# robotvisionmu/DenseMonoSLAM

Hardware: AMD Instinct MI355X
Metric: frames/sec ICP+RGB+fusion @640x480 (higher is better)
Workload: dtype f32; 1 GPU; TUM fr1/desk-like 640x480 full 3-level ICP+RGB tracking (SO3 + {10,5,4} GN iterations) + surfel index-map fusion; synthetic box-room RGB-D stream, loop closure off (--o), NID keyframing off (--nkf); cameras_per_gpu=1, n_pred=2, n_pred_project_passes=1, surfels_per_map=246557, surfels_total=246557, exchange=none (1 camera)

## Files before the change

densemonoslam_amd/capi.py:

```python
import ctypes as C
import os

import numpy as np

_HERE = os.path.dirname(os.path.abspath(__file__))
LIB_PATH = os.environ.get("DMS_LIB_PATH") or os.path.join(_HERE, "libdmslam_hip.so")

if not os.path.exists(LIB_PATH):
    raise ImportError(
        "densemonoslam_amd: %s is missing — build it with `make` (hipcc --offload-arch=gfx950) "
        "or `python -c 'import __graft_entry__ as g; g.build()'`; there is no CPU fallback" % LIB_PATH
    )

lib = C.CDLL(LIB_PATH)

DMS_OK = 0
NUM_PYRS = 3
MAX_SENSORS = 8


class Image2D(C.Structure):
    _fields_ = [("data", C.c_void_p), ("pitch", C.c_size_t), ("rows", C.c_int), ("cols", C.c_int)]


# ... 203 lines not shown
lib.dms_pyrDownGaussF.argtypes = [_I2, _I2, _P]
lib.dms_pyrDownUcharGauss.argtypes = [_I2, _I2, _P]
lib.dms_computeDerivativeImages.argtypes = [_I2, _I2, _I2, _P]
lib.dms_nid_workspace_bytes.argtypes = [C.c_int]
lib.dms_nid_workspace_bytes.restype = C.c_size_t
lib.dms_computeNIDImg.argtypes = [_I2, _I2, _I2, _I2, _I2, C.c_int, _P, C.c_size_t, C.POINTER(C.c_float), _P]
lib.dms_computeNIDDepth.argtypes = [_I2, _I2, _I2, C.c_int, C.c_float, _P, C.c_size_t, C.POINTER(C.c_float), _P]

lib.dms_fusion_wait_frame_done.argtypes = [_P, _P]
lib.dms_fusion_set_tracker_budget.argtypes = [_P, _I, _I]
lib.dms_fusion_get_tracker_budget.argtypes = [_P, C.POINTER(C.c_int), C.POINTER(C.c_int)]
lib.dms_fusion_allow_late_frame.argtypes = [_P, _I]
lib.dms_odometry_set_resident_budget.argtypes = [_P, _I, _I]
lib.dms_odometry_get_resident_budget.argtypes = [_P, C.POINTER(C.c_int), C.POINTER(C.c_int)]
lib.dms_exact_arith_selftest.argtypes = [_I, _F, C.POINTER(C.c_ulonglong), C.POINTER(C.c_uint)]

lib.dms_odometry_create.argtypes = [C.POINTER(_P), _I, _I, _F, _F, _F, _F, _F, _F]
lib.dms_odometry_destroy.argtypes = [_P]
lib.dms_odometry_set_mode.argtypes = [_P, _I, _I, _I, _I]
lib.dms_odometry_set_exec.argtypes = [_P, _I, _I, _I]
lib.dms_odometry_inject_timeout.argtypes = [_P, _I]
lib.dms_odometry_debug_set.argtypes = [_P, C.c_char_p, _I]
lib.dms_odometry_canon_retries.argtypes = [_P, _IP]
lib.dms_odometry_get_mode.argtypes = [_P, _IP, _IP, _IP]
lib.dms_odometry_get_level_shape.argtypes = [_P, _I, _IP, _IP, _IP]
lib.dms_debug_scalar_gn.argtypes = [_P, _P, _F, _P, _P, _P, _F, _F, _F, _F, _I, _P, _P, _P, _P, _P, _P]
lib.dms_debug_scalar_so3.argtypes = [_P, _P, _P, _F, _F, _F, _F, _P, _P, _P]
lib.dms_odometry_initICP_depth.argtypes = [_P, _I2, _F, _P]
lib.dms_odometry_initICP_maps.argtypes = [_P, _P, _P, _F, _P]
lib.dms_odometry_initICPModel.argtypes = [_P, _P, _P, _F, _FP, _P]
lib.dms_odometry_initRGB.argtypes = [_P, _I2, _P]
lib.dms_odometry_initRGBModel.argtypes = [_P, _I2, _P]
lib.dms_odometry_initFirstRGB.argtypes = [_P, _I2, _P]
lib.dms_odometry_initModelFused.argtypes = [_P, _P, _P, _P, _P, _P, _P, _P, C.c_int, _P, _P]
lib.dms_odometry_getIncrementalTransformation.argtypes = [_P, _FP, _FP, _I, _F, _I, _I, _I, _I, C.POINTER(TrackResult), _P]
lib.dms_odometry_track_async.argtypes = [_P, _FP, _FP, _I, _F, _I, _I, _I, _I, _P]
lib.dms_odometry_fetch_result.argtypes = [_P, C.POINTER(TrackResult), _P]
lib.dms_odometry_getCovariance.argtypes = [_P, C.POINTER(C.c_double)]
lib.dms_odometry_get_buffer.argtypes = [_P, _I, _I, _I2]
lib.dms_odometry_set_profiling.argtypes = [_P, _I]
lib.dms_odometry_get_kernel_time.argtypes = [_P, C.c_char_p, C.POINTER(C.c_double), _IP]
```

densemonoslam_amd/csrc/canon.hpp:

```cpp
#pragma once
#include "common.hpp"

namespace dms {
namespace canon {

constexpr int kMargin = 6;
constexpr int kEmin = -40;
constexpr int kEmax = 100;
constexpr int kRetryStep = 8;
constexpr int kMaxRetries = 16;

__host__ __device__ __forceinline__ int exp_of(float d) {
  if (!(d > 0.f) || !(d < 3.0e38f)) return -127;
  int e;
  (void)frexpf(d, &e);
  return e;
}
__host__ __device__ __forceinline__ int clamp_e(int e) { return e < kEmin ? kEmin : (e > kEmax ? kEmax : e); }

template <int N>
struct Layout {
  static constexpr int NP = N * (N + 3) / 2;
  static constexpr int NV = NP + 2;
  static constexpr int SLOTS = NV > 16 ? 32 : 16;
// ... 141 lines not shown
template <int SL>
__device__ __forceinline__ double tree_rest(const double (&o1)[SL / 2]) {
  const int lane = threadIdx.x & 63;
  double o2[SL / 4];
#pragma unroll
  for (int m = 0; m < SL / 4; ++m) o2[m] = swap16_add(o1[2 * m], o1[2 * m + 1]);
  double o3[SL / 8];
#pragma unroll
  for (int m = 0; m < SL / 8; ++m) o3[m] = sel_add<8>(o2[2 * m], o2[2 * m + 1], (lane & 8) != 0);
  double r;
  if constexpr (SL == 32) {
    double o4[2];
#pragma unroll
    for (int m = 0; m < 2; ++m) o4[m] = sel_add<4>(o3[2 * m], o3[2 * m + 1], (lane & 4) != 0);
    r = sel_add<2>(o4[0], o4[1], (lane & 2) != 0);
  } else {
    r = sel_add<4>(o3[0], o3[1], (lane & 4) != 0);
    r += mov_xor<2>(r);
  }
  r += mov_xor<1>(r);
  return r;
}

template <int N, int P>
__device__ __forceinline__ double wave_sum(const float (&rows)[P][N + 1], const bool (&found)[P], const double (*s_bias)[32]) {
  using Lay = Layout<N>;
  constexpr int SL = Lay::SLOTS;
  const int lane = threadIdx.x & 63;
  const double* bias = s_bias[lane >> 5];
  double r64[P][N + 1];
#pragma unroll
  for (int p = 0; p < P; ++p)
#pragma unroll
    for (int c = 0; c <= N; ++c) r64[p][c] = (double)rows[p][c];
  constexpr int G = 4, NG = (Lay::NV + G - 1) / G;
  double o1[SL / 2];
#pragma unroll
  for (int m = 0; m < SL / 2; ++m) o1[m] = 0.0;
  double cur[G], nxt[G];
#pragma unroll
  for (int h = 0; h < G; ++h) cur[h] = h < Lay::NV ? bias[h] : 0.0;
  round_down_begin();
#pragma unroll
  for (int g = 0; g < NG; ++g) {
#pragma unroll
    for (int h = 0; h < G; ++h) nxt[h] = ((g + 1) * G + h < Lay::NV) ? bias[(g + 1) * G + h] : 0.0;
#pragma unroll
    for (int p = 0; p < P; ++p) {
#pragma unroll
      for (int h = 0; h < G; ++h) {
        const int k = g * G + h;
        if (k <= Lay::NP)
          cur[h] = fma_down(r64[p][Lay::vi(k)], r64[p][Lay::vj(k)], cur[h]);
        else if (k == Lay::NP + 1)
          cur[h] += found[p] ? 1.0 : 0.0;
      }
    }
#pragma unroll
    for (int h = 0; h < G; h += 2)
      if (g * G + h < Lay::NV) o1[(g * G + h) / 2] = swap32_add(cur[h], cur[h + 1]);
#pragma unroll
    for (int h = 0; h < G; ++h) cur[h] = nxt[h];
  }
  round_down_end();
  return tree_rest<SL>(o1);
}

template <int N>
__device__ __forceinline__ void acc_init(double (&acc)[Layout<N>::NV], const double (*s_bias)[32]) {
  const double* bias = s_bias[(threadIdx.x & 63) >> 5];
#pragma unroll
// ... 58 lines not shown
```

densemonoslam_amd/csrc/scan.hpp:

```cpp
#pragma once
#include <hip/hip_runtime.h>

namespace dms {

__device__ __forceinline__ unsigned block_sum_u32(unsigned v) {
  __shared__ unsigned s_w[4];
  __shared__ unsigned s_tot;
  const int lane = threadIdx.x & 63, wid = threadIdx.x >> 6;
  for (int off = 32; off > 0; off >>= 1) v += __shfl_down(v, off, 64);
  if (lane == 0) s_w[wid] = v;
  __syncthreads();
  if (threadIdx.x == 0) s_tot = s_w[0] + s_w[1] + s_w[2] + s_w[3];
  __syncthreads();
  const unsigned t = s_tot;
  __syncthreads();
  return t;
}

__device__ __forceinline__ unsigned block_exclusive_rank(bool flag, unsigned& total) {
  __shared__ unsigned s_w[4];
  const int lane = threadIdx.x & 63, wid = threadIdx.x >> 6;
  const unsigned long long mask = __ballot(flag);
  const unsigned below = __popcll(mask & ((1ull << lane) - 1ull));
  __syncthreads();
  if (lane == 0) s_w[wid] = __popcll(mask);
  __syncthreads();
  unsigned base = 0;
  for (int w = 0; w < wid; ++w) base += s_w[w];
  total = s_w[0] + s_w[1] + s_w[2] + s_w[3];
  return base + below;
}

static __global__ __launch_bounds__(1024) void k_scan_blocks(const unsigned* __restrict__ counts, unsigned* __restrict__ offsets, int nb,
                                                      unsigned* __restrict__ out_count, unsigned cap, unsigned* __restrict__ out_count2) {
  __shared__ unsigned s_w[16];
  __shared__ unsigned s_carry;
  const int lane = threadIdx.x & 63, wid = threadIdx.x >> 6;
  if (threadIdx.x == 0) s_carry = 0;
  __syncthreads();
  for (int base = 0; base < nb; base += 1024) {
    const int i = base + threadIdx.x;
    const unsigned v = i < nb ? counts[i] : 0u;
    unsigned incl = v;
    for (int off = 1; off < 64; off <<= 1) {
      const unsigned t = __shfl_up(incl, off, 64);
      if (lane >= off) incl += t;
    }
    if (lane == 63) s_w[wid] = incl;
    __syncthreads();
    unsigned wbase = 0;
    for (int w = 0; w < wid; ++w) wbase += s_w[w];
    const unsigned carry = s_carry;
// ... 61 lines not shown
```

densemonoslam_amd/csrc/track.hip:

```cpp
#include <hip/hip_ext.h>
#include <math.h>

#include <map>
#include <string>
#include <vector>

#include "internal.hpp"
#include "host_util.hpp"
#include "pixel_ops.hpp"
#include "smallmath.hpp"
#include "gn_scalar.hpp"
#include "canon.hpp"
#include "pyr_body.hpp"
#include "frame_state.hpp"
#include "track_init.hpp"
#include "model_bodies.hpp"
#include "surfel.hpp"
#include "resident_rule.hpp"
#include <mutex>

namespace dms {

constexpr bool kTrackerFma = true;

struct Buf {
  void* p = nullptr;
  size_t pitch = 0;
  int rows = 0, cols = 0;
  dms_image2d img() const {
    dms_image2d i;
    i.data = p;
    i.pitch = pitch;
    i.rows = rows;
    i.cols = cols;
    return i;
  }
};

}

using namespace dms;
// ... 27 lines not shown
  float cx, cy, fx, fy, distThres, angleThres;
  float sobelScale, maxDepthDeltaRGB, maxDepthRGB;
  float minGrad[DMS_NUM_PYRS];
  char* arena = nullptr;
  size_t arena_bytes = 0;
  Buf depth_tmp[3], vmaps_g_prev[3], nmaps_g_prev[3], vmaps_curr[3], nmaps_curr[3];
  Buf lastDepth[3], nextDepth[3], lastImage[3], nextImage[3], lastNextImage[3];
  Buf nextdIdx[3], nextdIdy[3], nextGate[3], pointClouds[3], corresImg[3];
  struct LiveSet {
    Buf depth_tmp[3], vmaps_curr[3], nmaps_curr[3], nextImage[3], nextdIdx[3], nextdIdy[3], nextGate[3];
  };
  LiveSet ring[3];
  char* ring_arena = nullptr;
  bool ring_enabled = false;
  const void* deriv_of = nullptr;
  float* vmaps_tmp = nullptr;
  float* nmaps_tmp = nullptr;
  long long* part_icp = nullptr;
  long long* part_rgb = nullptr;
  long long* part_so3 = nullptr;
  int* part_cnt = nullptr;
  unsigned* tickets = nullptr;
  unsigned long long* ar = nullptr;
  int first_delay = -1;
  bool long_levels_resident = true;
  int first_delay_lvl[4] = {-1, -1, -1, -1};
  int first_delay_for(int nb, int stage) const { return dms::first_delay_for(nb, stage >= 0 && stage < 4 ? first_delay_lvl[stage] : -1, first_delay); }
  int depth_bias = 0;
  int exp_bias = 0;
  long long* prof = nullptr;
  TrackState* state = nullptr;
  TrackState* host_state = nullptr;
  bool profiling = false;
  bool profiling_level0_only = false;
  StageClock clock;
};

namespace dms {

__global__ void k_track_init(TrackState* st, Prior prior, const float* __restrict__ prior_pose16, float fx, float fy, float cx, float cy,
                             int so3, int first_level, unsigned long long* sync_words, int n_sync, int inject_timeout, unsigned* zero16) {
  track_init_body(blockIdx.x, gridDim.x, threadIdx.x, blockDim.x, st, prior, prior_pose16, fx, fy, cx, cy, so3, first_level, sync_words, n_sync,
                  inject_timeout, zero16);
}

__global__ __launch_bounds__(256) void k_track_init_pyr(TrackState* st, Prior prior, const float* __restrict__ prior_pose16, float fx, float fy,
// ... 588 lines not shown
  }
  if (ICP) canon::next_exponents<6>(s_icp, st->E_icp);
  if (RGB) canon::next_exponents<6>(s_rgb, st->E_rgb);
  st->have_E = 1;
  st->canon_retries += retries;
}

constexpr int kPWaves = kPB / kWave;
constexpr unsigned kSpinLimit = 1u << 22;

struct LevelArgs {
  int n_iter, level, level_below;
  int rgbOnly;
  float icpWeight;
  float fx, fy, cx, cy;
  unsigned long long* ar;
  int first_delay;
  long long* prof;
  int early_exit;
  int finalize, fin_rgb;
  float* pose16_out;
  FrameState* frame;
  float weightMultiplier;
};

constexpr int kArShards = 8;
constexpr int kArStride = 64;
constexpr int kArPairBase = kArShards * kArStride;
constexpr int kArPairStride = 16;
constexpr int kArWords = kArPairBase + kArShards * kArPairStride;
constexpr int kArSlotCnt = 0, kArSlotSig = 1;
constexpr int kArPool = 6;
constexpr int kArSetsPerKernel = kArRing + kArPool;
constexpr int kArSets = 4 * kArSetsPerKernel;

__device__ __forceinline__ unsigned long long pair_pack(unsigned long long v) { return (1ull << 58) + v; }

__device__ __forceinline__ void poll_pause(int n) {
  for (int i = 0; i < n; ++i) __builtin_amdgcn_s_sleep(1);
}
template <int STRIDE>
__device__ __forceinline__ bool ar_wait(const unsigned long long* w, int slot, bool mine, int nb, unsigned long long& fld_out, int* timeout) {
  unsigned spins = 0;
  for (;;) {
    unsigned long long arr = 0, fld = 0;
    if (mine) {
// ... 13 lines not shown
    }
    ++spins;
    if (spins > kSpinLimit || ((spins & 1023u) == 0u && __hip_atomic_load(timeout, __ATOMIC_RELAXED, __HIP_MEMORY_SCOPE_AGENT) == 1)) {
      __hip_atomic_store(timeout, 1, __ATOMIC_RELAXED, __HIP_MEMORY_SCOPE_AGENT);
      fld_out = 0;
      return false;
    }
    __builtin_amdgcn_s_sleep(1);
  }
}
__device__ __forceinline__ long long ar_total(unsigned long long fld, int nb) { return (long long)fld - (long long)nb * (1ll << 52); }

__device__ __forceinline__ constexpr unsigned se3_diag_mask() {
  unsigned m = 0;
  for (int c = 0; c <= 6; ++c) m |= 1u << canon::Layout<6>::diag(c);
  return m;
}
__device__ __forceinline__ constexpr unsigned so3_diag_mask() {
  unsigned m = 0;
  for (int c = 0; c <= 3; ++c) m |= 1u << canon::Layout<3>::diag(c);
  return m;
}

template <bool ICP, bool RGB, int P, bool EXIT>
__device__ __forceinline__ void gn_level_body(TrackState* st, const GnArgs& a, const LevelArgs& L, const int nb) {
  constexpr bool kFma = kTrackerFma;
  __shared__ sc::GnLocal s;
  __shared__ int s_redi[kPWaves][2];
  __shared__ double s_red[kPWaves][32];
  __shared__ double s_red2[2][kPWaves][32];
  __shared__ double s_bias[2][2][32];
  __shared__ int s_E[2][8];
  __shared__ float s_sums[64];
  __shared__ double s_comb[28];
  __shared__ float s_held[48];
  __shared__ int s_none;
  __shared__ int s_done;
  __shared__ int s_cs[2];
  __shared__ int s_viol;
  __shared__ int s_retries;
  __shared__ sc::KPre s_k[2];
  const int tid = threadIdx.x;
  int eb_icp = 0, eb_rgb = 0;
  __shared__ long long s_prof[16];
  if (tid < 16) s_prof[tid] = 0;
  long long pc = L.prof ? wall_clock64() : 0;
  auto phase = [&](int i) {
    if (L.prof && blockIdx.x == 0 && tid == 0) {
      const long long now = wall_clock64();
      s_prof[i] += now - pc;
      pc = now;
    }
  };

  if (L.finalize && L.frame && blockIdx.x == 0 && tid >= 64 && tid < 80) s_held[16 + tid - 64] = L.frame->lastPose[tid - 64];
  if (L.finalize && L.frame && blockIdx.x == 0 && tid >= 80 && tid < 84) s_held[12 + tid - 80] = L.frame->cur.pose[12 + tid - 80];
  if (tid == 0) {
    s_none = 0;
    s_retries = 0;
    s_done = st->level_done[L.level];
    for (int i = 0; i < 16; ++i) s.resultRt[i] = st->resultRt[i];
    for (int i = 0; i < 9; ++i) {
      s.Rprev[i] = st->Rprev[i];
      s.Rprev_inv[i] = st->Rprev_inv[i];
      s.Rcurr[i] = st->Rcurr[i];
      s.krkinv[i] = st->krkinv[i];
    }
    for (int i = 0; i < 3; ++i) {
      s.tprev[i] = st->tprev[i];
      s.tcurr[i] = st->tcurr[i];
      s.kt[i] = st->kt[i];
    }
    s.lastRGBError = st->lastRGBError;
    s.lastRGBCount = st->lastRGBCount;
    s.lastICPError = st->lastICPError;
    s.lastICPCount = st->lastICPCount;
    s.iters_run = st->iters_run[L.level];
    for (int i = 0; i < 36; ++i) s.lastA[i] = st->lastA[i];
    for (int i = 0; i < 6; ++i) s.lastb[i] = st->lastb[i];
    level_exponents(st, a, true, s_E[0], s_E[1]);
    s_k[0] = sc::kpre_of(L.fx, L.fy, L.cx, L.cy, L.level);
    s_k[1] = sc::kpre_of(L.fx, L.fy, L.cx, L.cy, L.level_below);
  }

  const int N = a.cols * a.rows;
  int idx[P], px[P], py[P];
  IcpOwn io[P];
  RgbOwn ro[P];
  short gx[P], gy[P];
#pragma unroll
  for (int p = 0; p < P; ++p) {
    idx[p] = (blockIdx.x * P + p) * kPB + tid;
    const int ic = idx[p] < N ? idx[p] : idx[p] % N;
    py[p] = ic / a.cols;
    px[p] = ic - py[p] * a.cols;
    if (ICP) io[p] = icp_load_own(a.maps, px[p], py[p], a.rows);
    if (RGB) {
      ro[p] = rgb_load_own_gated(a.rgb, px[p], py[p]);
      gx[p] = trow(a.rgb.dIdx, a.rgb.dI_pitch, py[p])[px[p]];
      gy[p] = trow(a.rgb.dIdy, a.rgb.dI_pitch, py[p])[px[p]];
    }
  }
  const float invFx = 1.0f / a.fx, invFy = 1.0f / a.fy;
  __syncthreads();
  if (s_done) return;
  if (tid < 64) {
    canon::write_bias<6>(s_E[tid >> 5], s_bias[tid >> 5], tid & 31);
    eb_icp = canon::value_exp<6>(s_E[0], tid & 31);
    eb_rgb = canon::value_exp<6>(s_E[1], tid & 31);
  }
  __syncthreads();

  bool ended = false;
  int pool_used = 0;
  bool on_pool = false;
  phase(0);
  for (int it = 0; it < L.n_iter;) {
    IcpParams ip;
    RgbResParams rp;
    if (ICP) ip = icp_params_of(s.Rcurr, s.tcurr, s.Rprev_inv, s.tprev, a);
    if (RGB) rp = rgb_params_of(s.krkinv, s.kt, a);
    const float lastErr = (it == 0) ? 3.402823466e+38F : s.lastRGBError;

    IcpProj ir[P];
    RgbProj rr[P];
    IcpModel im[P];
    RgbModel rm[P];
#pragma unroll
    for (int p = 0; p < P; ++p) {
      if (ICP) {
        ir[p] = icp_project<kFma>(ip, io[p]);
        im[p] = icp_load_model(a.maps, ir[p], a.rows);
      }
      if (RGB) {
        rr[p] = rgb_project<kFma>(rp, ro[p], px[p], py[p]);
        rm[p] = rgb_load_model(a.rgb, rr[p]);
      }
    }
    float rows[P][7];
    bool found[P];
    int cnt = 0, sig = 0;
    dms_dataterm c[P];
#pragma unroll
    for (int p = 0; p < P; ++p) {
      const bool live = idx[p] < N;
      if (RGB) {
        int d2;
        const bool ok = rgb_finish(rp, ro[p], rr[p], rm[p], px[p], py[p], c[p], d2) && live;
        if (!live) c[p].valid = 0;
        if (ok) {
          cnt += 1;
          sig += d2;
        }
      }
      if (ICP) {
        found[p] = icp_finish<kFma>(ip, io[p], ir[p], im[p], rows[p]);
        if (!live) {
          found[p] = false;
#pragma unroll
          for (int k = 0; k < 7; ++k) rows[p][k] = 0.f;
        }
      }
    }
    phase(1);
    const bool stamp = L.prof && L.level == 0 && it == L.n_iter / 2 && tid == 0;
    if (stamp) L.prof[48 + blockIdx.x * 8 + 0] = wall_clock64();
    const size_t set = (size_t)(on_pool ? kArRing + pool_used - 1 : it % kArRing) * kArWords;
    unsigned long long* arw = L.ar + set + (size_t)(blockIdx.x & (kArShards - 1)) * kArStride;
    const unsigned long long* arp = L.ar + set;
    unsigned long long* arq = L.ar + set + kArPairBase + (size_t)(blockIdx.x & (kArShards - 1)) * kArPairStride;
    int rgbSize = 0, sigma = 0;
    if (RGB) {
      const int lane = tid & 63, wid = tid >> 6;
      cnt = wave_sum_to_lane63_i(cnt);
      sig = wave_sum_to_lane63_i(sig);
      if (lane == 63) {
        s_redi[wid][0] = cnt;
        s_redi[wid][1] = sig;
      }
      __syncthreads();
      if (tid < 64) {
        const int t = row8_sum_i(tid < 16 ? s_redi[tid & 7][tid >> 3] : 0);
        const unsigned long long cb = (unsigned long long)(unsigned)__builtin_amdgcn_readlane(t, 0);
        const unsigned long long sb = (unsigned long long)(unsigned)__builtin_amdgcn_readlane(t, 8);
        if (tid < 2) __hip_atomic_fetch_add(arq + tid, pair_pack(tid == kArSlotCnt ? cb : sb), __ATOMIC_RELAXED, __HIP_MEMORY_SCOPE_AGENT);
      }
    }
    phase(2);
    double r_icp = 0.0;
    if (ICP) {
      if (RGB) {
        r_icp = canon::wave_sum<6, P>(rows, found, s_bias[0]);
      } else {
        const double p_icp = canon::block_sum<6, P, kPWaves>(rows, found, s_bias[0], s_red);
        if (tid < kSE3) __hip_atomic_fetch_add(arw + tid, canon::pack_word(canon::to_units(p_icp, eb_icp)), __ATOMIC_RELAXED, __HIP_MEMORY_SCOPE_AGENT);
      }
    }
    f3 cpt[P];
    float cinvz[P];
    if (RGB) {
#pragma unroll
      for (int p = 0; p < P; ++p) {
        const float z = rm[p].d0;
        cpt[p] = mk3((((float)c[p].zero_x - a.cx) * z) * invFx, (((float)c[p].zero_y - a.cy) * z) * invFy, z);
        cinvz[p] = rgb_row_invz(cpt[p]);
      }
    }
    if (RGB) {
      if (tid < 64) {
        unsigned long long fld;
        if (stamp) L.prof[48 + blockIdx.x * 8 + 4] = wall_clock64();
        ar_wait<kArPairStride>(arp + kArPairBase, tid, tid < 2, nb, fld, &st->sync_timeout);
        const int c0 = __builtin_amdgcn_readlane((int)fld, kArSlotCnt), s0 = __builtin_amdgcn_readlane((int)fld, kArSlotSig);
        if (tid == 0) {
          s_cs[0] = c0;
          s_cs[1] = s0;
        }
      }
      __syncthreads();
      rgbSize = s_cs[0];
      sigma = s_cs[1];
      phase(3);
      if (stamp) L.prof[48 + blockIdx.x * 8 + 1] = wall_clock64();
      if (L.rgbOnly && sc::rgbonly_break(sigma, rgbSize, lastErr)) {
        if (tid == 0) {
          double Rt[16];
          for (int i = 0; i < 16; ++i) Rt[i] = s.resultRt[i];
          sc::gn_params(Rt, s_k[1], s.krkinv, s.kt);
        }
        ended = true;
        break;
      }
      RgbStepParams p_;
      p_.sigma = L.rgbOnly ? -1.f : sc::sigma_val(sigma, rgbSize);
      p_.fx = a.fx;
      p_.fy = a.fy;
      p_.sobelScale = a.sobelScale;
#pragma unroll
      for (int p = 0; p < P; ++p) {
        RgbRowIn in;
        in.pt = cpt[p];
        in.gx = gx[p];
        in.gy = gy[p];
        rgb_row_finish<kFma>(p_, c[p], in, rows[p], cinvz[p], true);
        found[p] = c[p].valid != 0;
      }
      if (ICP) {
        const double r_rgb = canon::wave_sum<6, P>(rows, found, s_bias[1]);
        const int lane = tid & 63, wid = tid >> 6;
        if ((lane & 1) == 0) {
          const int sl = canon::slot_of_lane<32>(lane);
          s_red2[0][wid][sl] = r_icp;
          s_red2[1][wid][sl] = r_rgb;
        }
        __syncthreads();
        if (tid < 64 && (tid & 31) < kSE3) {
          double t = 0.0;
#pragma unroll
          for (int w = 0; w < kPWaves; ++w) t += s_red2[tid >> 5][w][tid & 31];
          __hip_atomic_fetch_add(arw + tid, canon::pack_word(canon::to_units(t, tid < 32 ? eb_icp : eb_rgb)), __ATOMIC_RELAXED, __HIP_MEMORY_SCOPE_AGENT);
        }
      } else {
      const double p_rgb = canon::block_sum<6, P, kPWaves>(rows, found, s_bias[1], s_red);
      if (tid < kSE3) __hip_atomic_fetch_add(arw + 32 + tid, canon::pack_word(canon::to_units(p_rgb, eb_rgb)), __ATOMIC_RELAXED, __HIP_MEMORY_SCOPE_AGENT);
      }
    }
    phase(4);
    if (stamp) L.prof[48 + blockIdx.x * 8 + 2] = wall_clock64();
    if (tid < 64) {
      const int k = tid & 31;
      const bool mine = k < kSE3 && (tid < 32 ? ICP : RGB);
      unsigned long long fld;
      poll_pause(L.first_delay);
      ar_wait<kArStride>(arp, tid, mine, nb, fld, &st->sync_timeout);
      const long long tot = ar_total(fld, nb);
      const float val = mine ? canon::from_units(tot, tid < 32 ? eb_icp : eb_rgb) : 0.f;
      s_sums[tid] = val;
      {
        const auto sw = __builtin_amdgcn_permlane32_swap(__float_as_uint(val), __float_as_uint(val), false, false);
        if (tid < 27) s_comb[tid] = sc::comb_entry(tid, ICP, RGB, L.icpWeight, val, __uint_as_float(sw[1]));
      }
      const bool bad = mine && ((se3_diag_mask() >> k) & 1u) && tot >= canon::kViolation;
      const unsigned long long any = __builtin_amdgcn_ballot_w64(bad);
      if (tid == 0) s_viol = ((any & 0xffffffffull) ? 1 : 0) | ((any >> 32) ? 2 : 0);
    }
    __syncthreads();
// ... 351 lines not shown
    mk(o->nmaps_g_prev[i], r * 3, w, 4);
    mk(o->vmaps_curr[i], r * 3, w, 4);
    mk(o->nmaps_curr[i], r * 3, w, 4);
    mk(o->lastDepth[i], r, w, 4);
    mk(o->nextDepth[i], r, w, 4);
    mk(o->lastImage[i], r, w, 1);
    mk(o->nextImage[i], r, w, 1);
    mk(o->lastNextImage[i], r, w, 1);
    mk(o->nextdIdx[i], r, w, 2);
    mk(o->nextdIdy[i], r, w, 2);
    mk(o->nextGate[i], r, w, 1);
    mk(o->pointClouds[i], r, w, 12);
    mk(o->corresImg[i], r, w, sizeof(dms_dataterm));
  }
  o->vmaps_tmp = (float*)c.take((size_t)W * H * 16);
  o->nmaps_tmp = (float*)c.take((size_t)W * H * 16);
  o->part_icp = (long long*)c.take((size_t)kRecWords * kMaxPartialBlocks * 8);
  o->part_rgb = (long long*)c.take((size_t)kRecWords * kMaxPartialBlocks * 8);
  o->part_so3 = (long long*)c.take((size_t)kRecWords * kMaxPartialBlocks * 8);
  o->part_cnt = (int*)c.take((size_t)2 * kMaxPartialBlocks * 4);
  o->tickets = (unsigned*)c.take(64);
  o->ar = (unsigned long long*)c.take((size_t)kArSets * kArWords * 8);
  o->prof = (long long*)c.take((3 * 16 + 256 * 8) * 8);
  o->state = (TrackState*)c.take(sizeof(TrackState));
}

bool timed(const dms_odometry* o, bool level0 = false) { return o->profiling && (level0 || !o->profiling_level0_only); }

float rgb_min_scale(const dms_odometry* o, int l) { return (float)(pow((double)o->minGrad[l], 2.0) / pow((double)o->sobelScale, 2.0)); }

int populateDepth(dms_odometry* o, Buf* destDepths, hipStream_t s) {
  int rc;
  dms_image2d d0 = destDepths[0].img();
  if ((rc = verticesToDepth(o->vmaps_tmp, &d0, o->maxDepthRGB, s))) return rc;
  for (int i = 0; i + 1 < DMS_NUM_PYRS; i++) {
    dms_image2d a = destDepths[i].img(), b = destDepths[i + 1].img();
    if ((rc = pyrDownGaussF(&a, &b, s))) return rc;
  }
  return DMS_OK;
}

int populateImage(const dms_image2d* rgba, Buf* destImages, hipStream_t s) {
  int rc;
  dms_image2d i0 = destImages[0].img();
  if ((rc = imageToIntensity(rgba, &i0, s))) return rc;
  for (int i = 0; i + 1 < DMS_NUM_PYRS; i++) {
// ... 63 lines not shown
  memset(o->host_state, 0, sizeof(TrackState));
  {
    const char* e = getenv("DMS_TRACK_MODE");
    o->resident = !(e && strcmp(e, "launches") == 0);
    e = getenv("DMS_TRACK_EARLY_EXIT");
    o->early_exit_force = e ? (e[0] != '0' ? 1 : 0) : -1;
    e = getenv("DMS_PERSIST_BLOCKS");
    if (e && atoi(e) > 0) o->persist_target = atoi(e);
    {
      int dev = 0, cus = 0, per_cu = 0;
      (void)hipGetDevice(&dev);
      if (hipDeviceGetAttribute(&cus, hipDeviceAttributeMultiprocessorCount, dev) != hipSuccess || cus <= 0) cus = 0;
      if (hipOccupancyMaxActiveBlocksPerMultiprocessor(&per_cu, (const void*)k_gn_level<true, true, 3, false>, kPB, 0) != hipSuccess) per_cu = 0;
      (void)hipGetLastError();
      o->max_resident_blocks = device_bound(cus, per_cu);
      if (o->max_resident_blocks <= 0) o->resident = false;
    }
    e = getenv("DMS_PERSIST_MAX_BLOCKS");
    o->max_resident_blocks = lowered_bound(o->max_resident_blocks, e ? atoi(e) : 0);
    e = getenv("DMS_AR_FIRST_DELAY");
    if (e && atoi(e) >= 0 && atoi(e) <= 1000) o->first_delay = atoi(e);
    e = getenv("DMS_TRACK_LONG_RESIDENT");
    if (e) o->long_levels_resident = atoi(e) != 0;
    e = getenv("DMS_AR_FIRST_DELAY_BY_LEVEL");
    if (e) {
      int v[4] = {-1, -1, -1, -1};
      if (sscanf(e, "%d,%d,%d,%d", &v[0], &v[1], &v[2], &v[3]) >= 1)
        for (int i = 0; i < 4; ++i)
          if (v[i] >= 0 && v[i] <= 1000) o->first_delay_lvl[i] = v[i];
    }
  }
  *out = o;
  return DMS_OK;
}

int dms_odometry_debug_set(dms_odometry* o, const char* key, int value) {
  DMS_REQUIRE(o && key, "null argument");
  if (strcmp(key, "exp_bias") == 0) {
    DMS_REQUIRE(value >= -100 && value <= 100, "exp_bias out of range");
    o->exp_bias = value;
    return DMS_OK;
  }
  if (strcmp(key, "depth_exp_bias") == 0) {
    DMS_REQUIRE(value >= 0 && value <= 100, "depth_exp_bias out of range");
    o->depth_bias = value;
    return DMS_OK;
  }
  DMS_REQUIRE(false, "unknown key");
}

int dms_odometry_set_resident_budget(dms_odometry* o, int max_blocks, int unchained) {
  DMS_REQUIRE(o && max_blocks >= 0, "bad argument");
  o->budget_cap = max_blocks;
  o->unchained_ok = unchained != 0 && max_blocks > 0;
  return DMS_OK;
}

int dms_odometry_get_resident_budget(dms_odometry* o, int* max_blocks, int* unchained) {
  DMS_REQUIRE(o, "null argument");
  if (max_blocks) *max_blocks = o->budget_cap;
  if (unchained) *unchained = o->unchained_ok ? 1 : 0;
  return DMS_OK;
}

int dms_odometry_get_mode(dms_odometry* o, int* resident, int* max_resident_blocks, int* fell_back) {
  DMS_REQUIRE(o, "null argument");
  if (resident) *resident = o->resident ? 1 : 0;
  if (max_resident_blocks) *max_resident_blocks = o->max_resident_blocks;
  if (fell_back) *fell_back = o->fell_back ? 1 : 0;
  return DMS_OK;
}
// ... 465 lines not shown
    a.exp_bias = o->exp_bias + o->depth_bias;
    return a;
  };
  auto level_args_of = [&](int l, int pnb) {
    LevelArgs L;
    L.n_iter = iterations[l];
    L.level = l;
    L.level_below = level_below_of(l);
    L.rgbOnly = rgbOnly ? 1 : 0;
    L.icpWeight = icpWeight;
    L.fx = o->fx;
    L.fy = o->fy;
    L.cx = o->cx;
    L.cy = o->cy;
    L.ar = o->ar + (size_t)(1 + l) * kArSetsPerKernel * kArWords;
    L.first_delay = o->first_delay_for(pnb, l);
    L.prof = (o->profiling && !o->profiling_level0_only) ? o->prof : nullptr;
    L.early_exit = o->early_exit_force >= 0 ? o->early_exit_force : (o->early_exit ? 1 : 0);
    L.finalize = (l == 0) ? 1 : 0;
    L.fin_rgb = rgb ? 1 : 0;
    L.pose16_out = frame ? const_cast<float*>(prior_pose16_dev) : nullptr;
    L.frame = frame;
    L.weightMultiplier = weightMultiplier;
    return L;
  };
  auto level_shape = [&](int l, int& pP, int& pnb) {
    const LevelShape sh = call_level_shape(budget_of(o), o->persist_target, iterations[l], o->resident, o->long_levels_resident, level_pixels(o, l));
    o->last_shape_P[l] = pP = sh.P;
    o->last_shape_nb[l] = pnb = sh.blocks;
  };

  if (so3) {
    const int L = 2;
    const Buf& li = o->lastNextImage[L];
    const Buf& ni = o->nextImage[L];
    const int nb = reduce_blocks_for(li.rows * li.cols);
    const int nbp = so3_resident_blocks(o);
    if (nbp > 0) {
      persist.begin();
      StageTimer t(o->clock, s, "so3_level", timed(o));
      SolveCam cam = {o->fx, o->fy, o->cx, o->cy};
      ex.nb_so3 = nbp;
      hipLaunchKernelGGL(k_so3_level, dim3(nbp + so3_rider_blocks(ex)), dim3(kPB), 0, s, o->state, (const unsigned char*)li.p, li.pitch,
                         (const unsigned char*)ni.p, ni.pitch, ni.cols, ni.rows, o->ar, cam, first_level, 10, o->exp_bias + o->depth_bias, o->first_delay_for(nbp, 3), ex);
      DMS_CHECK_LAUNCH();
    } else
    for (int i = 0; i < 10; ++i) {
      {
        StageTimer t(o->clock, s, "so3_pass", timed(o));
        SolveCam cam = {o->fx, o->fy, o->cx, o->cy};
        hipLaunchKernelGGL(k_so3_pass, dim3(nb), dim3(kBlock), 0, s, o->state, (const unsigned char*)li.p, li.pitch,
                           (const unsigned char*)ni.p, ni.pitch, ni.cols, ni.rows, o->part_so3, o->tickets, cam, i, i == 9 ? 1 : 0, first_level,
                           o->exp_bias + o->depth_bias);
        DMS_CHECK_LAUNCH();
      }
    }
  }

  bool finalized_in_kernel = false;
  for (int l = DMS_NUM_PYRS - 1; l >= 0; --l) {
    int pP = 1, pnb = 0;
    level_shape(l, pP, pnb);
    const bool persistent = pnb > 0;
    if (rgb && !persistent) {
      dms_camera k = {o->fx, o->fy, o->cx, o->cy};
      dms_image2d d = o->lastDepth[l].img(), c = o->pointClouds[l].img();
      if ((rc = projectToPointCloud(&d, &c, &k, l, s))) return rc;
    }
    if (iterations[l] == 0) continue;
    const GnArgs a = gn_args_of(l);
    const int nb = track_blocks_for(a.cols * a.rows);
    const int level_below = level_below_of(l);
    if (persistent) {
      const LevelArgs L = level_args_of(l, pnb);
      if (l == 0) finalized_in_kernel = true;
      persist.begin();
      static const char* const kLevelTimer[3] = {"gn_level0", "gn_level1", "gn_level2"};
      StageTimer t(o->clock, s, kLevelTimer[l], timed(o, l == 0));
      hipEvent_t done = (l == 0) ? persist.closing_event() : nullptr;
      if (icp && rgb)
        launch_gn_level<true, true>(pP, pnb, s, o->state, a, L, done);
      else if (icp)
        launch_gn_level<true, false>(pP, pnb, s, o->state, a, L, done);
      else
        launch_gn_level<false, true>(pP, pnb, s, o->state, a, L, done);
      DMS_CHECK_LAUNCH();
// ... 562 lines not shown
```

densemonoslam_amd/odometry.py:

```python
import ctypes as C

import numpy as np

from . import capi
from .capi import Camera, DeviceBuffer, DeviceImage, Image2D, TrackResult, check, lib


def _img(a):
    if isinstance(a, DeviceImage):
        return a
    return DeviceImage.from_array(a)


class ops:

    _ws = None

    @classmethod
    def workspace(cls):
        if cls._ws is None:
            cls._ws = DeviceBuffer(lib.dms_reduce_workspace_bytes())
        return cls._ws

    @staticmethod
# ... 209 lines not shown
        self.last = None

    def close(self):
        if getattr(self, "h", None):
            lib.dms_odometry_destroy(self.h)
            self.h = None

    def setMode(self, resident=-1, fp64_sums=-1, early_exit=-1, atomic_reduce=-1):
        check(lib.dms_odometry_set_exec(self.h, int(resident), int(early_exit), -1), "dms_odometry_set_exec")

    def getMode(self):
        a, b, c = C.c_int(0), C.c_int(0), C.c_int(0)
        check(lib.dms_odometry_get_mode(self.h, C.byref(a), C.byref(b), C.byref(c)), "dms_odometry_get_mode")
        return bool(a.value), b.value, bool(c.value)

    def levelShape(self, level):
        a, b, c = C.c_int(0), C.c_int(0), C.c_int(0)
        check(lib.dms_odometry_get_level_shape(self.h, int(level), C.byref(a), C.byref(b), C.byref(c)), "dms_odometry_get_level_shape")
        return a.value, b.value, bool(c.value)

    def setExpBias(self, bias):
        check(lib.dms_odometry_debug_set(self.h, b"exp_bias", int(bias)), "dms_odometry_debug_set")

    def canonRetries(self):
        n = C.c_int(0)
        check(lib.dms_odometry_canon_retries(self.h, C.byref(n)), "dms_odometry_canon_retries")
        return n.value

    def __del__(self):
        try:
            self.close()
        except Exception:
            pass

    @staticmethod
    def _dense(a):
        if isinstance(a, DeviceBuffer):
            return a, a.ptr
        if isinstance(a, DeviceImage):
            return a, a.buf.ptr
        if isinstance(a, int):
            return None, a
        arr = np.ascontiguousarray(a, np.float32)
        buf = DeviceBuffer(arr.nbytes).upload(arr)
        return buf, buf.ptr

# ... 79 lines not shown
```

include/dmslam.h:

```cpp
#ifndef DMSLAM_H_
#define DMSLAM_H_

#include <stddef.h>
#include <stdint.h>

#ifdef __cplusplus
extern "C" {
#endif

#define DMS_OK 0
#define DMS_ERR_INVALID_ARG (-1)
#define DMS_ERR_HIP (-2)
#define DMS_ERR_WORKSPACE (-3)
#define DMS_ERR_CAPACITY (-4)
#define DMS_ERR_STATE (-5)
#define DMS_ERR_TIMEOUT (-6)
#ifndef DMS_ERR_UNSUPPORTED
#define DMS_ERR_UNSUPPORTED (-7)
#endif
#define DMS_ERR_COMM (-9)

#define DMS_NUM_PYRS 3
#define DMS_MAX_SENSORS 8
#define DMS_REF_MAX_SENSORS 3
// ... 115 lines not shown

size_t dms_nid_workspace_bytes(int num_bins);
int dms_computeNIDImg(const dms_image2d* img_kf, const dms_image2d* img_kf_old, const dms_image2d* dmap_kf,
                      const dms_image2d* dmap_kf_old, const dms_image2d* img_curr, int num_bins,
                      void* workspace, size_t workspace_bytes, float* nid_host, dms_stream stream);
int dms_computeNIDDepth(const dms_image2d* dmap_kf, const dms_image2d* dmap_kf_old, const dms_image2d* dmap_curr,
                        int num_bins, float max_depth, void* workspace, size_t workspace_bytes,
                        float* nid_host, dms_stream stream);

typedef struct dms_odometry dms_odometry;

int dms_odometry_create(dms_odometry** out, int width, int height, float cx, float cy,
                        float fx, float fy, float distThresh, float angleThresh);
int dms_odometry_destroy(dms_odometry* o);
int dms_odometry_set_exec(dms_odometry* o, int resident, int early_exit, int coarse_launch);
int dms_odometry_set_resident_budget(dms_odometry* o, int max_blocks, int unchained);
int dms_odometry_get_resident_budget(dms_odometry* o, int* max_blocks, int* unchained);
int dms_odometry_set_mode(dms_odometry* o, int resident, int fp64_sums, int early_exit, int atomic_reduce);
int dms_odometry_fall_back_to_launches(dms_odometry* o);
int dms_odometry_get_mode(dms_odometry* o, int* resident, int* max_resident_blocks, int* fell_back);
int dms_odometry_get_level_shape(dms_odometry* o, int level, int* pixels_per_thread, int* blocks, int* resident);
int dms_odometry_inject_timeout(dms_odometry* o, int calls);
int dms_odometry_debug_set(dms_odometry* o, const char* key, int value);
int dms_odometry_canon_retries(dms_odometry* o, int* retries);
int dms_debug_scalar_gn(const float* sums_icp, const float* sums_rgb, float icpWeight, const float* Rprev, const float* tprev,
                        double* resultRt, float fx, float fy, float cx, float cy, int next_level, double* A, double* b,
                        float* Rcurr, float* tcurr, float* krkinv, float* kt);
int dms_debug_scalar_so3(const float* sums, float* R_lr, double* resultR, float fx, float fy, float cx, float cy,
                         float* imageBasis, float* kinv, float* krlr);

int dms_odometry_initICP_depth(dms_odometry* o, const dms_image2d* filteredDepth_u16,
                               float depthCutoff, dms_stream s);
int dms_odometry_initICP_maps(dms_odometry* o, const float* predictedVertices,
                              const float* predictedNormals, float depthCutoff, dms_stream s);
int dms_odometry_initICPModel(dms_odometry* o, const float* predictedVertices,
                              const float* predictedNormals, float depthCutoff,
                              const float* modelPose, dms_stream s);
int dms_odometry_initRGB(dms_odometry* o, const dms_image2d* rgba, dms_stream s);
int dms_odometry_initRGBModel(dms_odometry* o, const dms_image2d* rgba, dms_stream s);
int dms_odometry_initFirstRGB(dms_odometry* o, const dms_image2d* rgba, dms_stream s);
int dms_odometry_initModelFused(dms_odometry* o, const void* vertA, const void* normA, const void* rgbaA,
                                const void* vertB, const void* normB, const void* rgbaB, const int* use_b_dev,
                                int force_b_image, const float* modelPose16_dev, dms_stream s);

typedef struct dms_track_result {
  float trans[3];
// ... 33 lines not shown
```

Baseline: 2836 frames/s.

## Compact gated RGB pixels per block and interleave pixel ownership across blocks

In the persistent Gauss-Newton tracking body, each block now compacts its owned pixels that pass the RGB gate into a shared-memory list using a block-wide ballot rank. The RGB projection, finish and row build then run only over the number of occupied slots for the wave, dispatched through a compile-time slot count, and the canonical wave sum is cut to that count. Pixel ownership across blocks is also interleaved so the gated work spreads more evenly over blocks. The goal is to skip RGB arithmetic and loads for gated-out pixels in the iteration loop, in exchange for a one-time compaction pass, extra shared memory and more code variants from the templated slot dispatch.

```diff
diff --git a/densemonoslam_amd/capi.py b/densemonoslam_amd/capi.py
--- a/densemonoslam_amd/capi.py
+++ b/densemonoslam_amd/capi.py
@@ -249,6 +249,7 @@
 lib.dms_odometry_inject_timeout.argtypes = [_P, _I]
 lib.dms_odometry_debug_set.argtypes = [_P, C.c_char_p, _I]
 lib.dms_odometry_canon_retries.argtypes = [_P, _IP]
+lib.dms_odometry_get_rgb_compaction.argtypes = [_P, _I, _IP, _IP]
 lib.dms_odometry_get_mode.argtypes = [_P, _IP, _IP, _IP]
 lib.dms_odometry_get_level_shape.argtypes = [_P, _I, _IP, _IP, _IP]
 lib.dms_debug_scalar_gn.argtypes = [_P, _P, _F, _P, _P, _P, _F, _F, _F, _F, _I, _P, _P, _P, _P, _P, _P]
diff --git a/densemonoslam_amd/csrc/canon.hpp b/densemonoslam_amd/csrc/canon.hpp
--- a/densemonoslam_amd/csrc/canon.hpp
+++ b/densemonoslam_amd/csrc/canon.hpp
@@ -187,15 +187,16 @@
   return r;
 }
 
-template <int N, int P>
+template <int N, int P, int Q = P>
 __device__ __forceinline__ double wave_sum(const float (&rows)[P][N + 1], const bool (&found)[P], const double (*s_bias)[32]) {
+  static_assert(Q >= 1 && Q <= P, "wave_sum: 1 <= Q <= P");
   using Lay = Layout<N>;
   constexpr int SL = Lay::SLOTS;
   const int lane = threadIdx.x & 63;
   const double* bias = s_bias[lane >> 5];
-  double r64[P][N + 1];
-#pragma unroll
-  for (int p = 0; p < P; ++p)
+  double r64[Q][N + 1];
+#pragma unroll
+  for (int p = 0; p < Q; ++p)
 #pragma unroll
     for (int c = 0; c <= N; ++c) r64[p][c] = (double)rows[p][c];
   constexpr int G = 4, NG = (Lay::NV + G - 1) / G;
@@ -211,7 +212,7 @@
 #pragma unroll
     for (int h = 0; h < G; ++h) nxt[h] = ((g + 1) * G + h < Lay::NV) ? bias[(g + 1) * G + h] : 0.0;
 #pragma unroll
-    for (int p = 0; p < P; ++p) {
+    for (int p = 0; p < Q; ++p) {
 #pragma unroll
       for (int h = 0; h < G; ++h) {
         const int k = g * G + h;
diff --git a/densemonoslam_amd/csrc/scan.hpp b/densemonoslam_amd/csrc/scan.hpp
--- a/densemonoslam_amd/csrc/scan.hpp
+++ b/densemonoslam_amd/csrc/scan.hpp
@@ -17,17 +17,20 @@
   return t;
 }
 
+template <int NW = 4>
 __device__ __forceinline__ unsigned block_exclusive_rank(bool flag, unsigned& total) {
-  __shared__ unsigned s_w[4];
+  __shared__ unsigned s_w[NW];
   const int lane = threadIdx.x & 63, wid = threadIdx.x >> 6;
   const unsigned long long mask = __ballot(flag);
   const unsigned below = __popcll(mask & ((1ull << lane) - 1ull));
   __syncthreads();
   if (lane == 0) s_w[wid] = __popcll(mask);
   __syncthreads();
-  unsigned base = 0;
+  unsigned base = 0, tot = 0;
   for (int w = 0; w < wid; ++w) base += s_w[w];
-  total = s_w[0] + s_w[1] + s_w[2] + s_w[3];
+#pragma unroll
+  for (int w = 0; w < NW; ++w) tot += s_w[w];
+  total = tot;
   return base + below;
 }
 
diff --git a/densemonoslam_amd/csrc/track.hip b/densemonoslam_amd/csrc/track.hip
--- a/densemonoslam_amd/csrc/track.hip
+++ b/densemonoslam_amd/csrc/track.hip
@@ -2,6 +2,7 @@
 #include <math.h>
 
 #include <map>
+#include <type_traits>
 #include <string>
 #include <vector>
 
@@ -17,6 +18,8 @@
 #include "model_bodies.hpp"
 #include "surfel.hpp"
 #include "resident_rule.hpp"
+#include "track_ownership.hpp"
+#include "scan.hpp"
 #include <mutex>
 
 namespace dms {
@@ -90,6 +93,10 @@
   int* part_cnt = nullptr;
   unsigned* tickets = nullptr;
   unsigned long long* ar = nullptr;
+  unsigned* list_len = nullptr;
+  bool track_interleave = true;
+  bool rgb_compact = true;
+  bool last_rgb[DMS_NUM_PYRS] = {false, false, false};
   int first_delay = -1;
   bool long_levels_resident = true;
   int first_delay_lvl[4] = {-1, -1, -1, -1};
@@ -724,6 +731,9 @@
   float* pose16_out;
   FrameState* frame;
   float weightMultiplier;
+  int interleave;
+  int compact;
+  unsigned* list_len;
 };
 
 constexpr int kArShards = 8;
@@ -783,9 +793,30 @@
   return m;
 }
 
+static_assert(kOwnWaves == kPWaves && kOwnLanes == kWave, "track_ownership.hpp restates the block's shape");
+
+template <int P, typename F>
+__device__ __forceinline__ void for_slots(int q, F&& f) {
+  static_assert(P >= 1 && P <= 5, "for_slots: one case per slot");
+  if (q == 1) f(std::integral_constant<int, 1>());
+  if constexpr (P >= 2) {
+    if (q == 2) f(std::integral_constant<int, 2>());
+  }
+  if constexpr (P >= 3) {
+    if (q == 3) f(std::integral_constant<int, 3>());
+  }
+  if constexpr (P >= 4) {
+    if (q == 4) f(std::integral_constant<int, 4>());
+  }
+  if constexpr (P >= 5) {
+    if (q == 5) f(std::integral_constant<int, 5>());
+  }
+}
+
 template <bool ICP, bool RGB, int P, bool EXIT>
 __device__ __forceinline__ void gn_level_body(TrackState* st, const GnArgs& a, const LevelArgs& L, const int nb) {
   constexpr bool kFma = kTrackerFma;
+  constexpr bool kSkip = P <= 3;
   __shared__ sc::GnLocal s;
   __shared__ int s_redi[kPWaves][2];
   __shared__ double s_red[kPWaves][32];
@@ -801,6 +832,7 @@
   __shared__ int s_viol;
   __shared__ int s_retries;
   __shared__ sc::KPre s_k[2];
+  __shared__ unsigned s_list[RGB ? P * kPB : 1];
   const int tid = threadIdx.x;
   int eb_icp = 0, eb_rgb = 0;
   __shared__ long long s_prof[16];
@@ -845,32 +877,73 @@
   }
 
   const int N = a.cols * a.rows;
-  int idx[P], px[P], py[P];
+  bool live[P], keep[P];
+  unsigned own[P];
   IcpOwn io[P];
-  RgbOwn ro[P];
-  short gx[P], gy[P];
 #pragma unroll
   for (int p = 0; p < P; ++p) {
-    idx[p] = (blockIdx.x * P + p) * kPB + tid;
-    const int ic = idx[p] < N ? idx[p] : idx[p] % N;
-    py[p] = ic / a.cols;
-    px[p] = ic - py[p] * a.cols;
-    if (ICP) io[p] = icp_load_own(a.maps, px[p], py[p], a.rows);
-    if (RGB) {
-      ro[p] = rgb_load_own_gated(a.rgb, px[p], py[p]);
-      gx[p] = trow(a.rgb.dIdx, a.rgb.dI_pitch, py[p])[px[p]];
-      gy[p] = trow(a.rgb.dIdy, a.rgb.dI_pitch, py[p])[px[p]];
-    }
+    const int idx = owned_index(L.interleave != 0, (int)blockIdx.x, nb, P, p, tid);
+    const int ic = owned_shadow(idx, N);
+    const int y = ic / a.cols, x = ic - y * a.cols;
+    live[p] = idx < N;
+    own[p] = (unsigned)ic;
+    if (ICP) io[p] = icp_load_own(a.maps, x, y, a.rows);
+    keep[p] = false;
+    if (RGB) keep[p] = live[p] && (!L.compact || rgb_load_own_gated(a.rgb, x, y).gate);
   }
   const float invFx = 1.0f / a.fx, invFy = 1.0f / a.fy;
   __syncthreads();
-  if (s_done) return;
+  if (s_done) {
+    if (RGB && tid == 0 && L.list_len) L.list_len[blockIdx.x] = 0u;
+    return;
+  }
   if (tid < 64) {
     canon::write_bias<6>(s_E[tid >> 5], s_bias[tid >> 5], tid & 31);
     eb_icp = canon::value_exp<6>(s_E[0], tid & 31);
     eb_rgb = canon::value_exp<6>(s_E[1], tid & 31);
   }
   __syncthreads();
+
+  unsigned pxy[P], gxy[P], gi[P];
+  float d1[P];
+  auto own_of = [&](int q) {
+    RgbOwn o;
+    o.gate = (gi[q] >> 8) != 0u;
+    o.d1 = d1[q];
+    o.i1 = (unsigned char)(gi[q] & 0xffu);
+    return o;
+  };
+  int Qw = 0;
+  if (RGB) {
+    unsigned n = 0;
+#pragma unroll
+    for (int p = 0; p < P; ++p) {
+      unsigned tot;
+      const unsigned r = block_exclusive_rank<kPWaves>(keep[p], tot);
+      if (keep[p]) s_list[n + r] = own[p];
+      n += tot;
+    }
+    __syncthreads();
+    if (tid == 0 && L.list_len) L.list_len[blockIdx.x] = n;
+#pragma unroll
+    for (int q = 0; q < P; ++q) {
+      const unsigned e = (unsigned)(q * kPB + tid);
+      pxy[q] = gxy[q] = gi[q] = 0u;
+      d1[q] = 1.f;
+      if (e < n) {
+        const int i = (int)s_list[e];
+        const int y = i / a.cols, x = i - y * a.cols;
+        const RgbOwn o = rgb_load_own_gated(a.rgb, x, y);
+        const short gx = trow(a.rgb.dIdx, a.rgb.dI_pitch, y)[x], gy = trow(a.rgb.dIdy, a.rgb.dI_pitch, y)[x];
+        pxy[q] = (unsigned)x | ((unsigned)y << 16);
+        gxy[q] = (unsigned)(unsigned short)gx | ((unsigned)(unsigned short)gy << 16);
+        gi[q] = (unsigned)o.i1 | (o.gate ? 0x100u : 0u);
+        d1[q] = o.d1;
+      }
+    }
+    const unsigned first = (unsigned)(tid & ~(kWave - 1));
+    Qw = __builtin_amdgcn_readfirstlane(n > first ? (int)((n - first + kPB - 1) / kPB) : 0);
+  }
 
   bool ended = false;
   int pool_used = 0;
@@ -893,30 +966,40 @@
         ir[p] = icp_project<kFma>(ip, io[p]);
         im[p] = icp_load_model(a.maps, ir[p], a.rows);
       }
-      if (RGB) {
-        rr[p] = rgb_project<kFma>(rp, ro[p], px[p], py[p]);
-        rm[p] = rgb_load_model(a.rgb, rr[p]);
-      }
-    }
+    }
+    const int Qs = kSkip ? Qw : P;
+    if (RGB)
+      for_slots<P>(Qs, [&](auto qc) {
+#pragma unroll
+        for (int q = 0; q < decltype(qc)::value; ++q) {
+          rr[q] = rgb_project<kFma>(rp, own_of(q), (int)(pxy[q] & 0xffffu), (int)(pxy[q] >> 16));
+          rm[q] = rgb_load_model(a.rgb, rr[q]);
+        }
+      });
     float rows[P][7];
     bool found[P];
     int cnt = 0, sig = 0;
-    dms_dataterm c[P];
+    unsigned cz[P];
+    float cdiff[P];
+    if (RGB)
+      for_slots<P>(Qs, [&](auto qc) {
+#pragma unroll
+        for (int q = 0; q < decltype(qc)::value; ++q) {
+          int d2;
+          dms_dataterm c;
+          if (rgb_finish(rp, own_of(q), rr[q], rm[q], (int)(pxy[q] & 0xffffu), (int)(pxy[q] >> 16), c, d2)) {
+            cnt += 1;
+            sig += d2;
+          }
+          cz[q] = (unsigned)(unsigned short)c.zero_x | ((unsigned)(unsigned short)c.zero_y << 16) | (c.valid ? 0x80000000u : 0u);
+          cdiff[q] = c.diff;
+        }
+      });
 #pragma unroll
     for (int p = 0; p < P; ++p) {
-      const bool live = idx[p] < N;
-      if (RGB) {
-        int d2;
-        const bool ok = rgb_finish(rp, ro[p], rr[p], rm[p], px[p], py[p], c[p], d2) && live;
-        if (!live) c[p].valid = 0;
-        if (ok) {
-          cnt += 1;
-          sig += d2;
-        }
-      }
       if (ICP) {
         found[p] = icp_finish<kFma>(ip, io[p], ir[p], im[p], rows[p]);
-        if (!live) {
+        if (!live[p]) {
           found[p] = false;
 #pragma unroll
           for (int k = 0; k < 7; ++k) rows[p][k] = 0.f;
@@ -959,13 +1042,14 @@
     }
     f3 cpt[P];
     float cinvz[P];
-    if (RGB) {
-#pragma unroll
-      for (int p = 0; p < P; ++p) {
-        const float z = rm[p].d0;
-        cpt[p] = mk3((((float)c[p].zero_x - a.cx) * z) * invFx, (((float)c[p].zero_y - a.cy) * z) * invFy, z);
-        cinvz[p] = rgb_row_invz(cpt[p]);
-      }
+    auto cloud_point = [&](int q) {
+      const float z = rm[q].d0;
+      cpt[q] = mk3((((float)(short)(cz[q] & 0xffffu) - a.cx) * z) * invFx, (((float)(short)((cz[q] >> 16) & 0x7fffu) - a.cy) * z) * invFy, z);
+      cinvz[q] = rgb_row_invz(cpt[q]);
+    };
+    if (RGB && !kSkip) {
+#pragma unroll
+      for (int q = 0; q < P; ++q) cloud_point(q);
     }
     if (RGB) {
       if (tid < 64) {
@@ -997,17 +1081,29 @@
       p_.fx = a.fx;
       p_.fy = a.fy;
       p_.sobelScale = a.sobelScale;
-#pragma unroll
-      for (int p = 0; p < P; ++p) {
-        RgbRowIn in;
-        in.pt = cpt[p];
-        in.gx = gx[p];
-        in.gy = gy[p];
-        rgb_row_finish<kFma>(p_, c[p], in, rows[p], cinvz[p], true);
-        found[p] = c[p].valid != 0;
-      }
+      double r_rgb = 0.0;
+      for_slots<P>(Qs, [&](auto qc) {
+        constexpr int Q = decltype(qc)::value;
+#pragma unroll
+        for (int q = 0; q < Q; ++q) {
+          if (kSkip) cloud_point(q);
+          dms_dataterm c;
+          c.zero_x = (short)(cz[q] & 0xffffu);
+          c.zero_y = (short)((cz[q] >> 16) & 0x7fffu);
+          c.one_x = (short)(pxy[q] & 0xffffu);
+          c.one_y = (short)(pxy[q] >> 16);
+          c.diff = cdiff[q];
+          c.valid = (cz[q] >> 31) != 0u;
+          RgbRowIn in;
+          in.pt = cpt[q];
+          in.gx = (short)(gxy[q] & 0xffffu);
+          in.gy = (short)(gxy[q] >> 16);
+          rgb_row_finish<kFma>(p_, c, in, rows[q], cinvz[q], true);
+          found[q] = c.valid != 0;
+        }
+        r_rgb = canon::wave_sum<6, P, Q>(rows, found, s_bias[1]);
+      });
       if (ICP) {
-        const double r_rgb = canon::wave_sum<6, P>(rows, found, s_bias[1]);
         const int lane = tid & 63, wid = tid >> 6;
         if ((lane & 1) == 0) {
           const int sl = canon::slot_of_lane<32>(lane);
@@ -1022,7 +1118,7 @@
           __hip_atomic_fetch_add(arw + tid, canon::pack_word(canon::to_units(t, tid < 32 ? eb_icp : eb_rgb)), __ATOMIC_RELAXED, __HIP_MEMORY_SCOPE_AGENT);
         }
       } else {
-      const double p_rgb = canon::block_sum<6, P, kPWaves>(rows, found, s_bias[1], s_red);
+      const double p_rgb = canon::block_fold<6, kPWaves>(r_rgb, s_red);
       if (tid < kSE3) __hip_atomic_fetch_add(arw + 32 + tid, canon::pack_word(canon::to_units(p_rgb, eb_rgb)), __ATOMIC_RELAXED, __HIP_MEMORY_SCOPE_AGENT);
       }
     }
@@ -1420,6 +1516,7 @@
   o->tickets = (unsigned*)c.take(64);
   o->ar = (unsigned long long*)c.take((size_t)kArSets * kArWords * 8);
   o->prof = (long long*)c.take((3 * 16 + 256 * 8) * 8);
+  o->list_len = (unsigned*)c.take((size_t)DMS_NUM_PYRS * kMaxPersistBlocks * 4);
   o->state = (TrackState*)c.take(sizeof(TrackState));
 }
 
@@ -1529,6 +1626,10 @@
     if (e && atoi(e) >= 0 && atoi(e) <= 1000) o->first_delay = atoi(e);
     e = getenv("DMS_TRACK_LONG_RESIDENT");
     if (e) o->long_levels_resident = atoi(e) != 0;
+    e = getenv("DMS_TRACK_INTERLEAVE");
+    if (e) o->track_interleave = atoi(e) != 0;
+    e = getenv("DMS_RGB_COMPACT");
+    if (e) o->rgb_compact = atoi(e) != 0;
     e = getenv("DMS_AR_FIRST_DELAY_BY_LEVEL");
     if (e) {
       int v[4] = {-1, -1, -1, -1};
@@ -1553,7 +1654,35 @@
     o->depth_bias = value;
     return DMS_OK;
   }
+  if (strcmp(key, "track_interleave") == 0) {
+    o->track_interleave = value != 0;
+    return DMS_OK;
+  }
+  if (strcmp(key, "rgb_compact") == 0) {
+    o->rgb_compact = value != 0;
+    return DMS_OK;
+  }
   DMS_REQUIRE(false, "unknown key");
+}
+
+int dms_odometry_get_rgb_compaction(dms_odometry* o, int level, int* max_slots, int* entries) {
+  DMS_REQUIRE(o, "null argument");
+  DMS_REQUIRE(level >= 0 && level < DMS_NUM_PYRS, "bad level");
+  int q = 0, total = 0;
+  const int nb = o->last_rgb[level] ? o->last_shape_nb[level] : 0;
+  if (nb > 0) {
+    unsigned len[kMaxPersistBlocks];
+    DMS_HIP(hipDeviceSynchronize());
+    DMS_HIP(hipMemcpy(len, o->list_len + (size_t)level * kMaxPersistBlocks, (size_t)nb * 4, hipMemcpyDeviceToHost));
+    for (int b = 0; b < nb; ++b) {
+      const int slots = (int)((len[b] + kPB - 1) / kPB);
+      if (slots > q) q = slots;
+      total += (int)len[b];
+    }
+  }
+  if (max_slots) *max_slots = q;
+  if (entries) *entries = total;
+  return DMS_OK;
 }
 
 int dms_odometry_set_resident_budget(dms_odometry* o, int max_blocks, int unchained) {
@@ -2065,6 +2194,9 @@
     L.pose16_out = frame ? const_cast<float*>(prior_pose16_dev) : nullptr;
     L.frame = frame;
     L.weightMultiplier = weightMultiplier;
+    L.interleave = o->track_interleave ? 1 : 0;
+    L.compact = o->rgb_compact ? 1 : 0;
+    L.list_len = o->list_len + (size_t)l * kMaxPersistBlocks;
     return L;
   };
   auto level_shape = [&](int l, int& pP, int& pnb) {
@@ -2105,6 +2237,7 @@
     int pP = 1, pnb = 0;
     level_shape(l, pP, pnb);
     const bool persistent = pnb > 0;
+    o->last_rgb[l] = rgb && persistent && iterations[l] > 0;
     if (rgb && !persistent) {
       dms_camera k = {o->fx, o->fy, o->cx, o->cy};
       dms_image2d d = o->lastDepth[l].img(), c = o->pointClouds[l].img();
diff --git a/densemonoslam_amd/csrc/track_ownership.hpp b/densemonoslam_amd/csrc/track_ownership.hpp
--- /dev/null
+++ b/densemonoslam_amd/csrc/track_ownership.hpp
@@ -0,0 +1,22 @@
+#pragma once
+
+#if defined(__HIPCC__) || defined(__CUDACC__)
+#define DMS_OWN_HD __host__ __device__ __forceinline__
+#else
+#define DMS_OWN_HD inline
+#endif
+
+namespace dms {
+
+constexpr int kOwnLanes = 64;
+constexpr int kOwnWaves = 512 / 64;
+
+DMS_OWN_HD int owned_index(bool interleave, int b, int nb, int P, int p, int tid) {
+  const int w = tid / kOwnLanes, lane = tid % kOwnLanes;
+  const int seg = interleave ? (p * kOwnWaves + w) * nb + b : (b * P + p) * kOwnWaves + w;
+  return seg * kOwnLanes + lane;
+}
+
+DMS_OWN_HD int owned_shadow(int idx, int N) { return idx < N ? idx : idx % N; }
+
+}
diff --git a/densemonoslam_amd/odometry.py b/densemonoslam_amd/odometry.py
--- a/densemonoslam_amd/odometry.py
+++ b/densemonoslam_amd/odometry.py
@@ -255,6 +255,17 @@
     def setExpBias(self, bias):
         check(lib.dms_odometry_debug_set(self.h, b"exp_bias", int(bias)), "dms_odometry_debug_set")
 
+    def setOwnership(self, interleave=-1, compact=-1):
+        if interleave >= 0:
+            check(lib.dms_odometry_debug_set(self.h, b"track_interleave", int(interleave)), "dms_odometry_debug_set")
+        if compact >= 0:
+            check(lib.dms_odometry_debug_set(self.h, b"rgb_compact", int(compact)), "dms_odometry_debug_set")
+
+    def rgbCompaction(self, level):
+        q, n = C.c_int(0), C.c_int(0)
+        check(lib.dms_odometry_get_rgb_compaction(self.h, int(level), C.byref(q), C.byref(n)), "dms_odometry_get_rgb_compaction")
+        return q.value, n.value
+
     def canonRetries(self):
         n = C.c_int(0)
         check(lib.dms_odometry_canon_retries(self.h, C.byref(n)), "dms_odometry_canon_retries")
diff --git a/include/dmslam.h b/include/dmslam.h
--- a/include/dmslam.h
+++ b/include/dmslam.h
@@ -161,6 +161,7 @@
 int dms_odometry_get_level_shape(dms_odometry* o, int level, int* pixels_per_thread, int* blocks, int* resident);
 int dms_odometry_inject_timeout(dms_odometry* o, int calls);
 int dms_odometry_debug_set(dms_odometry* o, const char* key, int value);
+int dms_odometry_get_rgb_compaction(dms_odometry* o, int level, int* max_slots, int* entries);
 int dms_odometry_canon_retries(dms_odometry* o, int* retries);
 int dms_debug_scalar_gn(const float* sums_icp, const float* sums_rgb, float icpWeight, const float* Rprev, const float* tprev,
                         double* resultRt, float fx, float fy, float cx, float cy, int next_level, double* A, double* b,
```

After: 2944 frames/s (median of 6 runs). 3.8% higher.
